# korentomas/mlx-mcmc

Measured on NVIDIA B200. Metric: leapfrog_grad_evals_per_sec, higher is better.
Workload: dtype f32

## Files before the change

mlx_mcmc_b200/csrc/glm_rows.cuh:

```cuda
#pragma once
#include "glm.cuh"

namespace b2m {

__host__ __device__ inline float pow2_scale(float m) {
  if (!(m > 0.f) || !(m < 3.0e38f)) return 1.0f;
  int e;
  frexpf(m, &e);
  int k = 14 - e;
  if (k > 100) k = 100;
  if (k < -100) k = -100;
  return ldexpf(1.0f, k);
}

__device__ __forceinline__ void split_f16(float v, __half &hi, __half &lo) {
  hi = __float2half_rn(v);
  lo = __float2half_rn(v - __half2float(hi));
}

struct PackP {
  const float *beta0;
  const int *tf;
  float *thc;
  int Dtot, beta_off, D, Dp, sigma_param;
  float sigma_const, weight;
  const float *inv_col_scale;
  const unsigned *y0max_bits;
  float x_rownorm_max;
  int logit;
  __half *Bh, *Bl;
  float *inv_var, *a_unscale, *r_scale, *r_unscale;
  int n_peers;
  __half *peer_Bh[kMaxPeers], *peer_Bl[kMaxPeers];
  float4 *peer_meta[kMaxPeers];
};

__device__ __forceinline__ void pack16_row(const PackP &P, const float *__restrict__ th, int64_t row, int lane) {
  const bool live = th != nullptr;
  B2M_ASSERT(row >= 0 && P.Dp % 64 == 0 && P.D <= P.Dp && P.beta_off + P.D <= P.Dtot);
  const int *tf = P.tf;
  float amax = 0.f, n2 = 0.f;
  if (live) {
    if (tf) {
      float *tc = P.thc + row * P.Dtot;
      for (int d = lane; d < P.Dtot; d += 32) tc[d] = tf_constrain(tf[d], th[d]);
      __syncwarp();
      th = tc;
    }
    for (int d = lane; d < P.D; d += 32) {
      const float dl = __fsub_rn(th[P.beta_off + d], P.beta0[d]);
      amax = fmaxf(amax, fabsf(dl * P.inv_col_scale[d]));
      n2 = fmaf(dl, dl, n2);
    }
  }
  for (int o = 16; o > 0; o >>= 1) {
    amax = fmaxf(amax, __shfl_xor_sync(0xffffffffu, amax, o));
    n2 += __shfl_xor_sync(0xffffffffu, n2, o);
  }
  const float sa = pow2_scale(amax);
  const float sg = (live && P.sigma_param >= 0) ? th[P.sigma_param] : P.sigma_const;
  const float iv = 1.0f / (sg * sg);
  if (P.n_peers == 0) {
    for (int d = lane; d < P.Dp; d += 32) {
      float v = 0.f;
      if (live && d < P.D) v = __fsub_rn(th[P.beta_off + d], P.beta0[d]) * P.inv_col_scale[d] * sa;
      __half hi, lo;
      split_f16(v, hi, lo);
      P.Bh[row * P.Dp + d] = hi;
      P.Bl[row * P.Dp + d] = lo;
    }
    if (lane == 0) {
      P.inv_var[row] = iv;
      P.a_unscale[row] = 1.0f / sa;
      if (P.r_scale) {
        const float bound = P.logit ? fabsf(P.weight)
                                    : (__uint_as_float(*P.y0max_bits) + sqrtf(n2) * P.x_rownorm_max) * fabsf(iv * P.weight);
        const float sr = pow2_scale(bound);
        P.r_scale[row] = sr;
        P.r_unscale[row] = 1.0f / sr;
      }
    }
  } else {
    for (int d = 2 * lane; d < P.Dp; d += 64) {
      float v0 = 0.f, v1 = 0.f;
      if (live && d < P.D) v0 = __fsub_rn(th[P.beta_off + d], P.beta0[d]) * P.inv_col_scale[d] * sa;
      if (live && d + 1 < P.D) v1 = __fsub_rn(th[P.beta_off + d + 1], P.beta0[d + 1]) * P.inv_col_scale[d + 1] * sa;
      const __half2 hi = __floats2half2_rn(v0, v1);
      const float2 hf = __half22float2(hi);
      const __half2 lo = __floats2half2_rn(v0 - hf.x, v1 - hf.y);
#pragma unroll
      for (int s = 0; s < kMaxPeers; ++s)
        if (s < P.n_peers) {
          *reinterpret_cast<__half2 *>(P.peer_Bh[s] + row * P.Dp + d) = hi;
          *reinterpret_cast<__half2 *>(P.peer_Bl[s] + row * P.Dp + d) = lo;
        }
    }
    if (lane < P.n_peers) P.peer_meta[lane][row] = make_float4(iv, 1.0f / sa, n2, 0.f);
  }
}

struct FinishP {
  int has_prior;
  int Dtot, beta_off, D, Dp, sigma_param;
  float sigma_const, weight;
  int N;
  int logit;
  int n_tiles;
  const float *ss_part;
  const float *G;
  int g_splits;
  int64_t Cp;
  const float *r_unscale;
  const float *inv_col_scale;
  const int *tf;
  const float *thc;
  int gram;
  const double *gb;
  const float *beta0;
  const float *a_unscale;
  const float *g_unscale;
};

__device__ __forceinline__ float gram_row(const FinishP &F, const float *__restrict__ th, int64_t c, float ivw,
                                          float *__restrict__ gr, int lane) {
  const int D = F.D, Dp = F.Dp, beta_off = F.beta_off;
  const int64_t stride = F.Cp * (int64_t)Dp;
  const float *__restrict__ Gr = F.G + c * Dp;
  const float au = F.a_unscale ? F.a_unscale[c] : 1.0f;
  const int step = (D & 3) == 0 ? 4 : 1;
  double acc = 0.0;
  for (int j0 = step * lane; j0 < D; j0 += 32 * step) {
    float p[4] = {0.f, 0.f, 0.f, 0.f};
    if (step == 4) {
#pragma unroll 4
      for (int s = 0; s < F.g_splits; ++s) {
        const float4 t = *reinterpret_cast<const float4 *>(Gr + s * stride + j0);
        p[0] += t.x; p[1] += t.y; p[2] += t.z; p[3] += t.w;
      }
    } else {
#pragma unroll 4
      for (int s = 0; s < F.g_splits; ++s) p[0] += Gr[s * stride + j0];
    }
#pragma unroll
    for (int e = 0; e < 4; ++e) {
      if (e >= step) break;
      const int j = j0 + e;
      const float pj = F.g_unscale ? p[e] * (au * F.g_unscale[j]) : p[e];
      const double bj = F.gb[j];
      const float dl = __fsub_rn(th[beta_off + j], F.beta0[j]);
      acc += (double)dl * ((double)pj - 2.0 * bj);
      if (gr) gr[beta_off + j] = (float)(bj - (double)pj) * ivw;
    }
  }
  for (int o = 16; o > 0; o >>= 1) acc += __shfl_xor_sync(0xffffffffu, acc, o);
  return (float)(F.gb[Dp] + acc);
}

__device__ __forceinline__ void finish_row(const FinishP &F, const SModel &sm, const float *__restrict__ th, int64_t c,
                                           int64_t c_batch, float *__restrict__ logp_out, float *__restrict__ gr, int lane) {
  B2M_ASSERT(c >= 0 && c < F.Cp && F.g_splits >= 0 && F.n_tiles >= 1);
  const float *thu = th;
  if (F.tf) th = F.thc + c_batch * F.Dtot;
  const int Dtot = F.Dtot, D = F.D, Dp = F.Dp, beta_off = F.beta_off, sigma_param = F.sigma_param;
  const int64_t Cp = F.Cp;
  const float *__restrict__ G = F.G;
  const float sg = sigma_param >= 0 ? th[sigma_param] : F.sigma_const;
  const float iv = 1.0f / (sg * sg);
  const float weight = F.weight;
  float ss = 0.f;
  if (F.gram) {
    ss = gram_row(F, th, c, iv * weight, gr, lane);
    if (gr) {
      for (int d = lane; d < Dtot; d += 32)
        if (d < beta_off || d >= beta_off + D) gr[d] = d == sigma_param ? weight * (ss * iv - (float)F.N) / sg : 0.f;
    }
    __syncwarp();
  } else {
    for (int t = lane; t < F.n_tiles; t += 32) ss += F.ss_part[(int64_t)t * Cp + c];
    for (int o = 16; o > 0; o >>= 1) ss += __shfl_xor_sync(0xffffffffu, ss, o);
  }
  float lp = F.logit ? weight * ss : weight * ((float)F.N * (-kHalfLog2Pi - logf(sg)) - 0.5f * ss * iv);
  const bool vec4 = !F.gram && gr && sigma_param < 0 && (Dtot & 3) == 0 && (beta_off & 3) == 0 && (D & 3) == 0 &&
                    ((reinterpret_cast<uintptr_t>(gr) | reinterpret_cast<uintptr_t>(G)) & 15) == 0;
  if (vec4) {
    const float ru = F.r_unscale ? F.r_unscale[c] : 1.0f;
    for (int d = 4 * lane; d < Dtot; d += 128) {
      float4 v = make_float4(0.f, 0.f, 0.f, 0.f);
      if (d >= beta_off && d < beta_off + D) {
        const float4 *g4 = reinterpret_cast<const float4 *>(G + (int64_t)c * Dp + (d - beta_off));
        const int64_t stride4 = (Cp * (int64_t)Dp) >> 2;
#pragma unroll 8
        for (int s = 0; s < F.g_splits; ++s) {
          const float4 t = g4[(int64_t)s * stride4];
          v.x += t.x; v.y += t.y; v.z += t.z; v.w += t.w;
        }
        if (F.r_unscale) {
          const float4 ic = *reinterpret_cast<const float4 *>(F.inv_col_scale + (d - beta_off));
          v.x *= ru * ic.x; v.y *= ru * ic.y; v.z *= ru * ic.z; v.w *= ru * ic.w;
        }
      }
      *reinterpret_cast<float4 *>(gr + d) = v;
    }
    __syncwarp();
  } else if (gr && !F.gram) {
#pragma unroll 2
    for (int d = lane; d < Dtot; d += 32) {
      float v = 0.f;
      if (d >= beta_off && d < beta_off + D) {
#pragma unroll 8
        for (int s = 0; s < F.g_splits; ++s) v += G[((int64_t)s * Cp + c) * Dp + (d - beta_off)];
        if (F.r_unscale) v *= F.r_unscale[c] * F.inv_col_scale[d - beta_off];
      }
      if (d == sigma_param) v = weight * (ss * iv - (float)F.N) / sg;
      gr[d] = v;
    }
    __syncwarp();
  }
  float pl = 0.f;
  const int n_terms = F.has_prior ? sm.n_terms : 0;
  for (int t = 0; t < n_terms; ++t) {
    const b2m_term &T = sm.terms[t];
    float acc = 0.f, ax = 0.f, a0 = 0.f, a1 = 0.f;
    if (T.dist == B2M_NORMAL && T.x.kind == B2M_OP_PARAMVEC && T.p0.kind == B2M_OP_CONST && T.p1.kind == B2M_OP_CONST) {
      const float p0 = T.p0.c, p1 = T.p1.c, var = p1 * p1, base = -kHalfLog2Pi - logf(p1), w = T.weight;
      const float *__restrict__ xv = th + T.x.a;
      float *__restrict__ gv = gr ? gr + T.x.a : nullptr;
      if ((T.length & 3) == 0 && ((reinterpret_cast<uintptr_t>(xv) | reinterpret_cast<uintptr_t>(gv)) & 15) == 0) {
        for (int n = 4 * lane; n < T.length; n += 128) {
          const float4 x4 = *reinterpret_cast<const float4 *>(xv + n);
          const float z0 = x4.x - p0, z1 = x4.y - p0, z2 = x4.z - p0, z3 = x4.w - p0;
          acc += base - (0.5f * (z0 * z0)) / var;
          acc += base - (0.5f * (z1 * z1)) / var;
          acc += base - (0.5f * (z2 * z2)) / var;
          acc += base - (0.5f * (z3 * z3)) / var;
          if (gv) {
            float4 g4 = *reinterpret_cast<float4 *>(gv + n);
            g4.x += w * (-(z0 / var)); g4.y += w * (-(z1 / var)); g4.z += w * (-(z2 / var)); g4.w += w * (-(z3 / var));
            *reinterpret_cast<float4 *>(gv + n) = g4;
          }
        }
      } else {
#pragma unroll 4
        for (int n = lane; n < T.length; n += 32) {
          const float z = xv[n] - p0;
          acc += base - (0.5f * (z * z)) / var;
          if (gv) gv[n] += w * (-(z / var));
        }
      }
      for (int o = 16; o > 0; o >>= 1) acc += __shfl_xor_sync(0xffffffffu, acc, o);
      pl += w * acc;
      __syncwarp();
      continue;
    }
    for (int n = lane; n < T.length; n += 32) {
      const float x = op_fetch(T.x, n, th, 1, sm), p0 = op_fetch(T.p0, n, th, 1, sm), p1 = op_fetch(T.p1, n, th, 1, sm);
      Elem e = dist_eval<true>(T.dist, x, p0, p1, T.k0, T.k1, T.k2);
      acc += e.lp;
      if (gr) {
        if (T.x.kind == B2M_OP_PARAM) ax += e.dx; else if (T.x.kind == B2M_OP_PARAMVEC) gr[T.x.a + n] += T.weight * e.dx;
        if (T.p0.kind == B2M_OP_PARAM) a0 += e.d0; else if (T.p0.kind == B2M_OP_PARAMVEC) gr[T.p0.a + n] += T.weight * e.d0;
        if (T.p1.kind == B2M_OP_PARAM) a1 += e.d1; else if (T.p1.kind == B2M_OP_PARAMVEC) gr[T.p1.a + n] += T.weight * e.d1;
      }
    }
    for (int o = 16; o > 0; o >>= 1) {
      acc += __shfl_xor_sync(0xffffffffu, acc, o);
      ax += __shfl_xor_sync(0xffffffffu, ax, o);
      a0 += __shfl_xor_sync(0xffffffffu, a0, o);
      a1 += __shfl_xor_sync(0xffffffffu, a1, o);
    }
// ... 29 lines not shown
```

mlx_mcmc_b200/csrc/glm_samplers.cu:

```cuda
#include <stdlib.h>

#include <chrono>
#include <string>
#include <vector>

#include "glm_rows.cuh"

namespace b2m {

constexpr int WPB = 4;

__device__ __forceinline__ float warp_sum(float v) {
  for (int o = 16; o > 0; o >>= 1) v += __shfl_xor_sync(0xffffffffu, v, o);
  return v;
}

__device__ __forceinline__ void normals4(uint64_t seed, uint64_t gchain, uint32_t giter, int group, float out[4]) {
  const uint4 w = Philox::draw(seed, gchain, giter, 1u + (uint32_t)group);
  box_muller(w.x, w.y, out[0], out[1]);
  box_muller(w.z, w.w, out[2], out[3]);
}

__device__ __noinline__ void fill_momentum(float *p, int D, const float *inj, uint64_t seed, uint64_t gchain, uint32_t giter,
                                           uint4 w0, int lane, const float *__restrict__ im = nullptr) {
// ... 253 lines not shown
  layout(real);
  const unsigned grid = (unsigned)((C + WPB - 1) / WPB);
  int rc = glm_logp_grad(gm, a.theta, C, a.logp, nullptr, st, true);
  for (int it = 0; it < a.n_iter && !rc; ++it) {
    if (it > 0 && (it & 15) == 0) rc = glm_recenter(gm, a.theta, C, st);
    mh_propose_kernel<<<grid, 32 * WPB, 0, st>>>(a, qn, D, it);
    rc = glm_logp_grad(gm, qn, C, lpn, nullptr, st);
    mh_accept_kernel<<<grid, 32 * WPB, 0, st>>>(a, qn, lpn, D, it, gm.tf);
    g_launches += 2;
  }
  cudaError_t e = cudaStreamSynchronize(st);
  if (rc) return rc;
  B2M_CHECK_CUDA(e);
  B2M_CHECK_CUDA(cudaGetLastError());
  return 0;
}

struct NutsBufs {
  float *g, *fq, *fp, *fg;
  float *slots;
  int n_slots;
  int *lo, *hi, *cand;
  int *leaf_slot;
  int *sub_c;
  int *st_f, *st_c;
  float *lp, *clp, *h0, *log_slice, *flp, *sclp, *feps, *heps;
  int *n, *s, *v, *leaf, *building, *sub_n, *sub_na, *sub_s, *alpha_cnt, *depth;
  double *alpha_sum, *sub_alpha;
  float *st_clp;
  int *st_n, *st_na;
  double *st_alpha;
  int *n_active;
  int *active;
  float *alpha_it;
  double *eps_it;
  int *state;
  int *iter;
  int *fin;
  int *live;
  int *n_done;
  double *pool;
  const int *tf;
};

__device__ __noinline__ void vcopy(float *__restrict__ dst, const float *__restrict__ src, int D, int lane) {
  if ((D & 3) == 0 && ((reinterpret_cast<uintptr_t>(dst) | reinterpret_cast<uintptr_t>(src)) & 15) == 0) {
// ... 97 lines not shown
    W.feps[c] = (float)((double)v * eps);
    W.heps[c] = (float)(0.5 * ((double)v * eps));
    W.leaf[c] = 0;
    W.building[c] = 1;
  }
}

__global__ void __launch_bounds__(32 * WPB) nuts_doubling_begin_kernel(b2m_nuts_args A, NutsBufs W, int D, int it, int j) {
  CHAIN_PROLOGUE(A.n_chains)
  nuts_doubling_begin_dev(A, W, D, c, lane, it, j);
}

__device__ __forceinline__ void nuts_leaf_pre_dev(const b2m_nuts_args &A, const NutsBufs &W, int D, int64_t c, int lane) {
  if (!W.building[c]) return;
  const size_t o = (size_t)c * D;
  const float he = W.heps[c], fe = W.feps[c];
  float *__restrict__ fq = W.fq + o, *__restrict__ fp = W.fp + o;
  const int s = W.leaf_slot[c];
  const float *__restrict__ sq = slot_row(W, D, c, s, 0), *__restrict__ sp = slot_row(W, D, c, s, 1),
                            *__restrict__ sg = slot_row(W, D, c, s, 2);
  if (const float *__restrict__ im = A.inv_mass) {
#pragma unroll 4
    for (int d = lane; d < D; d += 32) {
      const float pv = __fadd_rn(sp[d], __fmul_rn(he, sg[d]));
      fp[d] = pv;
      fq[d] = __fadd_rn(sq[d], __fmul_rn(fe, im[d] * pv));
    }
    return;
  }
  if ((D & 3) == 0 && ((reinterpret_cast<uintptr_t>(fq) | reinterpret_cast<uintptr_t>(fp) | reinterpret_cast<uintptr_t>(sq) |
                        reinterpret_cast<uintptr_t>(sp) | reinterpret_cast<uintptr_t>(sg)) & 15) == 0) {
    for (int d = 4 * lane; d < D; d += 128) {
      const float4 g4 = *reinterpret_cast<const float4 *>(sg + d);
      float4 p4 = *reinterpret_cast<const float4 *>(sp + d), q4 = *reinterpret_cast<const float4 *>(sq + d);
      p4.x = __fadd_rn(p4.x, __fmul_rn(he, g4.x)); p4.y = __fadd_rn(p4.y, __fmul_rn(he, g4.y));
      p4.z = __fadd_rn(p4.z, __fmul_rn(he, g4.z)); p4.w = __fadd_rn(p4.w, __fmul_rn(he, g4.w));
      q4.x = __fadd_rn(q4.x, __fmul_rn(fe, p4.x)); q4.y = __fadd_rn(q4.y, __fmul_rn(fe, p4.y));
      q4.z = __fadd_rn(q4.z, __fmul_rn(fe, p4.z)); q4.w = __fadd_rn(q4.w, __fmul_rn(fe, p4.w));
      *reinterpret_cast<float4 *>(fp + d) = p4;
      *reinterpret_cast<float4 *>(fq + d) = q4;
    }
    return;
  }
#pragma unroll 4
  for (int d = lane; d < D; d += 32) {
    const float pv = __fadd_rn(sp[d], __fmul_rn(he, sg[d]));
    fp[d] = pv;
    fq[d] = __fadd_rn(sq[d], __fmul_rn(fe, pv));
  }
}

__global__ void __launch_bounds__(32 * WPB) nuts_leaf_pre_kernel(b2m_nuts_args A, NutsBufs W, int D) {
  CHAIN_PROLOGUE(A.n_chains)
  nuts_leaf_pre_dev(A, W, D, c, lane);
}

__device__ __forceinline__ void nuts_leaf_post_dev(const b2m_nuts_args &A, const NutsBufs &W, int D, int64_t c, int lane, int it, int j) {
  if (!W.building[c]) return;
  const int64_t C = A.n_chains;
  const uint64_t gchain = (uint64_t)(A.chain_offset + c);
  const uint32_t giter = (uint32_t)(A.iter_offset + it);
  const size_t row = (size_t)it * C + c;
  const size_t o = (size_t)c * D;
  const int MD = A.max_tree_depth;
  const bool ref_compat = A.compat == B2M_COMPAT_REFERENCE;
  const float *fq = W.fq + o, *fp = W.fp + o, *fg = W.fg + o;
  const float he = W.heps[c];
  const int i = W.leaf[c];
  unsigned live = (1u << W.lo[c]) | (1u << W.hi[c]) | (1u << W.cand[c]);
  for (int k = 0; k < j; ++k)
    if ((i >> k) & 1) live |= (1u << W.st_f[(size_t)k * C + c]) | (1u << W.st_c[(size_t)k * C + c]);
  const int L = __ffs(~live) - 1;
  B2M_ASSERT(L >= 0 && L < W.n_slots);
  float *__restrict__ lq = slot_row(W, D, c, L, 0), *__restrict__ lp = slot_row(W, D, c, L, 1), *__restrict__ lg = slot_row(W, D, c, L, 2);
  float k0 = 0.f, k1 = 0.f;
  {
    int d = lane;
    if ((D & 3) == 0 && ((reinterpret_cast<uintptr_t>(fq) | reinterpret_cast<uintptr_t>(fp) | reinterpret_cast<uintptr_t>(fg) |
                          reinterpret_cast<uintptr_t>(lq) | reinterpret_cast<uintptr_t>(lp) | reinterpret_cast<uintptr_t>(lg)) & 15) == 0) {
      for (int e = 4 * lane; e < D; e += 128) {
        const float4 q4 = *reinterpret_cast<const float4 *>(fq + e), g4 = *reinterpret_cast<const float4 *>(fg + e);
        float4 p4 = *reinterpret_cast<const float4 *>(fp + e);
        p4.x = __fadd_rn(p4.x, __fmul_rn(he, g4.x)); p4.y = __fadd_rn(p4.y, __fmul_rn(he, g4.y));
        p4.z = __fadd_rn(p4.z, __fmul_rn(he, g4.z)); p4.w = __fadd_rn(p4.w, __fmul_rn(he, g4.w));
        k0 = fmaf(p4.x, p4.x, k0); k1 = fmaf(p4.y, p4.y, k1); k0 = fmaf(p4.z, p4.z, k0); k1 = fmaf(p4.w, p4.w, k1);
        *reinterpret_cast<float4 *>(lq + e) = q4; *reinterpret_cast<float4 *>(lp + e) = p4; *reinterpret_cast<float4 *>(lg + e) = g4;
      }
      d = D;
    }
    for (; d + 32 < D; d += 64) {
      const float q0 = fq[d], q1 = fq[d + 32], g0 = fg[d], g1 = fg[d + 32];
      const float p0 = __fadd_rn(fp[d], __fmul_rn(he, g0)), p1 = __fadd_rn(fp[d + 32], __fmul_rn(he, g1));
      k0 = fmaf(p0, p0, k0); k1 = fmaf(p1, p1, k1);
      lq[d] = q0; lq[d + 32] = q1; lp[d] = p0; lp[d + 32] = p1; lg[d] = g0; lg[d + 32] = g1;
    }
    for (; d < D; d += 32) {
      const float q0 = fq[d], g0 = fg[d];
      const float p0 = __fadd_rn(fp[d], __fmul_rn(he, g0));
      k0 = fmaf(p0, p0, k0);
      lq[d] = q0; lp[d] = p0; lg[d] = g0;
    }
  }
  float kin = 0.5f * warp_sum(k0 + k1);
  __syncwarp();
  if (A.inv_mass) kin = kinetic_w(lp, D, lane, A.inv_mass);
  const float flp = W.flp[c], h0 = W.h0[c], log_slice = W.log_slice[c];
  const float h1 = -flp + kin;
  const int n1 = (log_slice <= -h1) ? 1 : 0;
  const bool s1 = log_slice < (1000.0f - h1);
  float a1 = expf(-h1 + h0);
  if (a1 != a1) a1 = ref_compat ? 1.0f : 0.0f;
  a1 = fminf(a1, 1.0f);
  const int v = W.v[c];
  B2M_ASSERT(j >= 0 && j < A.max_tree_depth && i >= 0 && i < (1 << j) && (v == 1 || v == -1));
  if (lane == 0) {
    A.n_leaves[c] += 1;
    if (!s1) A.n_diverge[c] += 1;
  }
  float sub_clp = flp;
  int sub_n = n1, sub_na = 1;
  bool sub_s = s1;
  double sub_alpha = (double)a1;
  int sf = L, sc = L;
  int k = 0;
  bool finished = false;
  while (true) {
    if (k == j) { finished = true; break; }
    const size_t ss = (size_t)k * C + c;
// ... 27 lines not shown
    } else {
      if (sub_s) {
        if (lane == 0) {
          W.st_f[ss] = sf; W.st_c[ss] = sc;
          W.st_clp[ss] = sub_clp; W.st_n[ss] = sub_n; W.st_na[ss] = sub_na; W.st_alpha[ss] = sub_alpha;
        }
        break;
      }
      ++k;
    }
  }
  if (lane == 0) {
    W.leaf_slot[c] = L;
    if (finished) {
      W.building[c] = 0;
      W.sub_c[c] = sc;
      W.sclp[c] = sub_clp; W.sub_n[c] = sub_n; W.sub_na[c] = sub_na; W.sub_s[c] = sub_s ? 1 : 0; W.sub_alpha[c] = sub_alpha;
    } else {
      W.leaf[c] = i + 1;
    }
  }
}

__global__ void __launch_bounds__(32 * WPB) nuts_leaf_post_kernel(b2m_nuts_args A, NutsBufs W, int D, int it, int j) {
  CHAIN_PROLOGUE(A.n_chains)
  nuts_leaf_post_dev(A, W, D, c, lane, it, j);
}

__device__ __forceinline__ void nuts_doubling_end_dev(const b2m_nuts_args &A, const NutsBufs &W, int D, int64_t c, int lane, int it, int j) {
  if (!W.s[c]) return;
  const uint64_t gchain = (uint64_t)(A.chain_offset + c);
  const uint32_t giter = (uint32_t)(A.iter_offset + it);
  const size_t row = (size_t)it * A.n_chains + c;
  const int v = W.v[c];
  int lo = W.lo[c], hi = W.hi[c];
  if (v == 1) hi = W.leaf_slot[c];
  else        lo = W.leaf_slot[c];
  const int sub_n = W.sub_n[c], sub_s = W.sub_s[c];
  const int n = W.n[c];
  int took = 0;
  if (sub_s) {
    float ut;
    if (A.inj_take) ut = A.inj_take[row * A.max_tree_depth + j];
    else ut = u01(Philox::draw(A.seed, gchain, giter, SLOT_NUTS_DOUBLING + j).y);
    const double pr = fmin(1.0, (double)sub_n / fmax((double)n, 1.0));
    if ((double)ut < pr) took = 1;
// ... 110 lines not shown
    h_bar = (1.0 - eta) * h_bar + eta * (A.target_accept - mean_alpha);
    float log_eps = __fsub_rn(mu, (float)((sqrt(m + 1.0) / 0.05) * h_bar));
    log_eps = fmaxf(fminf(log_eps, 10.0f), -10.0f);
    const double eps = (double)expf(log_eps);
    const double wgt = pow(m + 1.0, -0.75);
    eps_bar = (double)expf((float)(wgt * log(eps) + (1.0 - wgt) * log(eps_bar)));
    eps_sh = eps; hbar_sh = h_bar; ebar_sh = eps_bar;
  }
  __syncthreads();
  for (int64_t c = threadIdx.x; c < C; c += 1024) {
    A.step_size[c] = eps_sh;
    A.da_state[c * 3 + 0] = hbar_sh;
    A.da_state[c * 3 + 1] = ebar_sh;
  }
}

static void nuts_layout(Arena &A, NutsBufs &W, int64_t C, int D, int MD) {
  const size_t cd = (size_t)C * D;
  float **vecs[] = {&W.g, &W.fq, &W.fp, &W.fg};
  for (auto v : vecs) A.take(v, cd);
  static_assert(2 * B2M_MAX_TREE_DEPTH + 2 <= 32, "the free-slot search keeps the live slots in a 32-bit mask");
  W.n_slots = 2 * MD + 2;
  A.take(&W.slots, cd * 3 * W.n_slots);
  float **fs[] = {&W.lp, &W.clp, &W.h0, &W.log_slice, &W.flp, &W.sclp, &W.feps, &W.heps};
  for (auto v : fs) A.take(v, C);
  int **is[] = {&W.n, &W.s, &W.v, &W.leaf, &W.building, &W.sub_n, &W.sub_na, &W.sub_s, &W.alpha_cnt, &W.depth,
                &W.lo, &W.hi, &W.cand, &W.leaf_slot, &W.sub_c};
  for (auto v : is) A.take(v, C);
  A.take(&W.st_f, (size_t)C * MD); A.take(&W.st_c, (size_t)C * MD);
  A.take(&W.alpha_sum, C); A.take(&W.sub_alpha, C);
  A.take(&W.st_clp, (size_t)C * MD); A.take(&W.st_n, (size_t)C * MD); A.take(&W.st_na, (size_t)C * MD);
  A.take(&W.st_alpha, (size_t)C * MD);
  A.take(&W.n_active, 1);
  A.take(&W.active, C);
  A.take(&W.alpha_it, C);
  A.take(&W.eps_it, C);
  A.take(&W.state, C); A.take(&W.iter, C); A.take(&W.fin, C); A.take(&W.live, C);
  A.take(&W.n_done, 1);
  A.take(&W.pool, 4);
}

__device__ __forceinline__ void nuts_tick_dev(const b2m_nuts_args &A, const NutsBufs &W, int D, int64_t c, int lane) {
  B2M_ASSERT(c >= 0 && c < A.n_chains);
  const int st = W.state[c];
  B2M_ASSERT(st >= 0 && st <= 2);
  if (st == 2) return;
  int it = W.iter[c];
  B2M_ASSERT(it >= 0 && it < A.n_iter);
  B2M_ASSERT(W.depth[c] >= 0 && W.depth[c] <= A.max_tree_depth);
  bool begin_transition = st == 0;
  int begin_doubling = -1;
  if (st != 0) {
    const int j = W.depth[c];
    nuts_leaf_post_dev(A, W, D, c, lane, it, j);
    __syncwarp();
    if (!W.building[c]) {
      nuts_doubling_end_dev(A, W, D, c, lane, it, j);
      __syncwarp();
      if (W.s[c] && W.depth[c] < A.max_tree_depth) {
        begin_doubling = W.depth[c];
      } else {
        nuts_end_dev(A, W, D, c, lane, it);
        __syncwarp();
        ++it;
        if (lane == 0) { W.iter[c] = it; W.fin[c] = 1; }
        if (it >= A.n_iter) {
          if (lane == 0) { W.state[c] = 2; W.live[c] = 0; atomicAdd(W.n_done, 1); }
          return;
        }
        begin_transition = true;
      }
    }
  }
  if (begin_transition) {
    nuts_begin_dev(A, W, D, c, lane, it);
    __syncwarp();
    begin_doubling = 0;
    if (st == 0 && lane == 0) W.state[c] = 1;
  }
  if (begin_doubling >= 0) {
    nuts_doubling_begin_dev(A, W, D, c, lane, it, begin_doubling);
    __syncwarp();
  }
  nuts_leaf_pre_dev(A, W, D, c, lane);
}

__global__ void __launch_bounds__(32 * WPB) nuts_tick_kernel(b2m_nuts_args A, NutsBufs W, int D, int64_t c_base, int64_t c_end) {
  const int lane = threadIdx.x & 31;
  const int64_t c = c_base + (int64_t)blockIdx.x * WPB + (threadIdx.x >> 5);
  if (c >= c_end) return;
  nuts_tick_dev(A, W, D, c, lane);
}

struct StateP {
  FinishP F;
  PackP P;
  const int *idx;
  int64_t n_rows;
  int64_t n_pad;
  int64_t row_base;
  int do_finish, do_tick_pack;
  unsigned *blk_counter;
  volatile long long *h_prog;
  long long tick;
  int peer, nranks, rank;
  unsigned long long wait_seq, seq;
  const unsigned long long *gflag;
  unsigned long long *bflag_peer[kMaxPeers];
  long long *done_peer[kMaxPeers];
  int *err;
};

constexpr int kProgRing = 8;
constexpr long long kSpinTimeout = 20000000000ll;

__device__ __forceinline__ unsigned long long ld_acquire_sys(const unsigned long long *p) {
  unsigned long long v;
  asm volatile("ld.acquire.sys.global.u64 %0, [%1];" : "=l"(v) : "l"(p) : "memory");
  return v;
}
__device__ __forceinline__ void st_release_sys(unsigned long long *p, unsigned long long v) {
  asm volatile("st.release.sys.global.u64 [%0], %1;" ::"l"(p), "l"(v) : "memory");
}
__device__ __forceinline__ void spin_until(const unsigned long long *flag, unsigned long long want, int *err) {
  const long long t0 = clock64();
  while (ld_acquire_sys(flag) < want) {
    if (*reinterpret_cast<volatile int *>(err)) return;
    if (clock64() - t0 > kSpinTimeout) { *reinterpret_cast<volatile int *>(err) = 1; __threadfence_system(); return; }
    __nanosleep(64);
  }
}

__global__ void __launch_bounds__(32 * WPB, 7) nuts_state_kernel(b2m_nuts_args A, NutsBufs W, int D, KModel prior, StateP S) {
  extern __shared__ __align__(16) unsigned char smem[];
  SModel sm;
  sm.n_terms = 0;
  if (S.do_finish && S.F.has_prior) model_to_smem(prior, smem, sm);
  const int lane = threadIdx.x & 31, warp = threadIdx.x >> 5;
  if (S.peer && S.do_finish) {
    if ((int)threadIdx.x < S.nranks) spin_until(S.gflag + threadIdx.x, S.wait_seq, S.err);
    __syncthreads();
  }
  const int64_t r = (int64_t)blockIdx.x * WPB + warp;
  if (r < S.n_rows) {
    const int64_t row = S.row_base + r;
    const int64_t c = S.idx ? S.idx[row] : row;
    B2M_ASSERT(c >= 0 && c < A.n_chains && row >= 0 && (S.peer || row < S.n_pad));
    if (S.do_finish) {
      finish_row(S.F, sm, W.fq + c * D, S.peer ? r : row, row, W.flp + c, W.fg + c * D, lane);
      __syncwarp();
    }
    if (S.do_tick_pack) {
      nuts_tick_dev(A, W, D, c, lane);
      __syncwarp();
      pack16_row(S.P, W.fq + c * D, row, lane);
    }
  } else if (r < S.n_pad && S.do_tick_pack) {
    pack16_row(S.P, nullptr, S.row_base + r, lane);
  }
  if (!S.do_tick_pack) return;
  if (S.peer) __threadfence_system(); else __threadfence();
  __syncwarp();
  int last_warp = 0;
  if (lane == 0) {
    const unsigned prev = atomicAdd(S.blk_counter, 1u);
    last_warp = prev == gridDim.x * WPB - 1;
    if (last_warp) *S.blk_counter = 0;
  }
  last_warp = __shfl_sync(0xffffffffu, last_warp, 0);
  if (!last_warp) return;
  __threadfence();
  const long long n_done = *reinterpret_cast<volatile int *>(W.n_done);
  if (S.peer) {
    if (lane < S.nranks) {
      *reinterpret_cast<volatile long long *>(S.done_peer[lane]) = n_done;
      __threadfence_system();
      st_release_sys(S.bflag_peer[lane], S.seq);
    }
// ... 495 lines not shown
```

Baseline: 31.65 million.

## Fuse NUTS leaf close into gradient finish and leaf open into pack

After: 36.45 million (median of 6 runs). 1.15x the previous value.

```diff
diff --git a/mlx_mcmc_b200/csrc/glm_rows.cuh b/mlx_mcmc_b200/csrc/glm_rows.cuh
--- a/mlx_mcmc_b200/csrc/glm_rows.cuh
+++ b/mlx_mcmc_b200/csrc/glm_rows.cuh
@@ -17,6 +17,16 @@
   hi = __float2half_rn(v);
   lo = __float2half_rn(v - __half2float(hi));
 }
+
+__device__ __forceinline__ float leaf_kick(float p, float he, float g) { return __fadd_rn(p, __fmul_rn(he, g)); }
+__device__ __forceinline__ float leaf_drift(float q, float fe, float v) { return __fadd_rn(q, __fmul_rn(fe, v)); }
+__device__ __forceinline__ float pack_coef(float th, float b0, float ics, float sa) { return __fsub_rn(th, b0) * ics * sa; }
+__device__ __forceinline__ float gram_elem(float pj, double bj, float dl, float ivw, double &acc) {
+  acc += (double)dl * ((double)pj - 2.0 * bj);
+  return (float)(bj - (double)pj) * ivw;
+}
+__device__ __forceinline__ float normal_prior_lp(float z, float base, float var) { return base - (0.5f * (z * z)) / var; }
+__device__ __forceinline__ float normal_prior_dx(float z, float var, float w) { return w * (-(z / var)); }
 
 struct PackP {
   const float *beta0;
@@ -63,7 +73,7 @@
   if (P.n_peers == 0) {
     for (int d = lane; d < P.Dp; d += 32) {
       float v = 0.f;
-      if (live && d < P.D) v = __fsub_rn(th[P.beta_off + d], P.beta0[d]) * P.inv_col_scale[d] * sa;
+      if (live && d < P.D) v = pack_coef(th[P.beta_off + d], P.beta0[d], P.inv_col_scale[d], sa);
       __half hi, lo;
       split_f16(v, hi, lo);
       P.Bh[row * P.Dp + d] = hi;
@@ -83,8 +93,8 @@
   } else {
     for (int d = 2 * lane; d < P.Dp; d += 64) {
       float v0 = 0.f, v1 = 0.f;
-      if (live && d < P.D) v0 = __fsub_rn(th[P.beta_off + d], P.beta0[d]) * P.inv_col_scale[d] * sa;
-      if (live && d + 1 < P.D) v1 = __fsub_rn(th[P.beta_off + d + 1], P.beta0[d + 1]) * P.inv_col_scale[d + 1] * sa;
+      if (live && d < P.D) v0 = pack_coef(th[P.beta_off + d], P.beta0[d], P.inv_col_scale[d], sa);
+      if (live && d + 1 < P.D) v1 = pack_coef(th[P.beta_off + d + 1], P.beta0[d + 1], P.inv_col_scale[d + 1], sa);
       const __half2 hi = __floats2half2_rn(v0, v1);
       const float2 hf = __half22float2(hi);
       const __half2 lo = __floats2half2_rn(v0 - hf.x, v1 - hf.y);
@@ -96,6 +106,55 @@
         }
     }
     if (lane < P.n_peers) P.peer_meta[lane][row] = make_float4(iv, 1.0f / sa, n2, 0.f);
+  }
+}
+
+__device__ __forceinline__ bool open_pack_ok(const PackP &P, int Dtot) {
+  return P.n_peers == 0 && !P.r_scale && !P.tf && P.sigma_param < 0 && P.beta_off == 0 && P.D == Dtot && (Dtot & 3) == 0 &&
+         ((reinterpret_cast<uintptr_t>(P.beta0) | reinterpret_cast<uintptr_t>(P.inv_col_scale)) & 15) == 0;
+}
+
+__device__ __forceinline__ void open_pack16_row(const PackP &P, const float *__restrict__ sq, const float *__restrict__ sp,
+                                                const float *__restrict__ sg, float he, float fe, float *__restrict__ q,
+                                                float *__restrict__ p, int64_t row, int lane) {
+  const int D = P.D;
+  float amax = 0.f;
+  for (int d = 4 * lane; d < D; d += 128) {
+    const float4 g4 = *reinterpret_cast<const float4 *>(sg + d), b4 = *reinterpret_cast<const float4 *>(P.beta0 + d),
+                 c4 = *reinterpret_cast<const float4 *>(P.inv_col_scale + d);
+    float4 p4 = *reinterpret_cast<const float4 *>(sp + d), q4 = *reinterpret_cast<const float4 *>(sq + d);
+    p4.x = leaf_kick(p4.x, he, g4.x); p4.y = leaf_kick(p4.y, he, g4.y);
+    p4.z = leaf_kick(p4.z, he, g4.z); p4.w = leaf_kick(p4.w, he, g4.w);
+    q4.x = leaf_drift(q4.x, fe, p4.x); q4.y = leaf_drift(q4.y, fe, p4.y);
+    q4.z = leaf_drift(q4.z, fe, p4.z); q4.w = leaf_drift(q4.w, fe, p4.w);
+    *reinterpret_cast<float4 *>(p + d) = p4;
+    *reinterpret_cast<float4 *>(q + d) = q4;
+    amax = fmaxf(amax, fabsf(__fsub_rn(q4.x, b4.x) * c4.x)); amax = fmaxf(amax, fabsf(__fsub_rn(q4.y, b4.y) * c4.y));
+    amax = fmaxf(amax, fabsf(__fsub_rn(q4.z, b4.z) * c4.z)); amax = fmaxf(amax, fabsf(__fsub_rn(q4.w, b4.w) * c4.w));
+  }
+  for (int o = 16; o > 0; o >>= 1) amax = fmaxf(amax, __shfl_xor_sync(0xffffffffu, amax, o));
+  const float sa = pow2_scale(amax);
+  for (int d = 4 * lane; d < P.Dp; d += 128) {
+    float v[4] = {0.f, 0.f, 0.f, 0.f};
+    if (d < D) {
+      const float4 q4 = *reinterpret_cast<const float4 *>(q + d), b4 = *reinterpret_cast<const float4 *>(P.beta0 + d),
+                   c4 = *reinterpret_cast<const float4 *>(P.inv_col_scale + d);
+      v[0] = pack_coef(q4.x, b4.x, c4.x, sa); v[1] = pack_coef(q4.y, b4.y, c4.y, sa);
+      v[2] = pack_coef(q4.z, b4.z, c4.z, sa); v[3] = pack_coef(q4.w, b4.w, c4.w, sa);
+    }
+    __half hi[4], lo[4];
+#pragma unroll
+    for (int e = 0; e < 4; ++e) split_f16(v[e], hi[e], lo[e]);
+    *reinterpret_cast<uint2 *>(P.Bh + row * P.Dp + d) =
+        make_uint2(__half_as_ushort(hi[0]) | (unsigned)__half_as_ushort(hi[1]) << 16,
+                   __half_as_ushort(hi[2]) | (unsigned)__half_as_ushort(hi[3]) << 16);
+    *reinterpret_cast<uint2 *>(P.Bl + row * P.Dp + d) =
+        make_uint2(__half_as_ushort(lo[0]) | (unsigned)__half_as_ushort(lo[1]) << 16,
+                   __half_as_ushort(lo[2]) | (unsigned)__half_as_ushort(lo[3]) << 16);
+  }
+  if (lane == 0) {
+    P.inv_var[row] = 1.0f / (P.sigma_const * P.sigma_const);
+    P.a_unscale[row] = 1.0f / sa;
   }
 }
 
@@ -121,6 +180,10 @@
   const float *g_unscale;
 };
 
+__device__ __forceinline__ float gram_unscale(const FinishP &F, float pj, float au, int j) {
+  return F.g_unscale ? pj * (au * F.g_unscale[j]) : pj;
+}
+
 __device__ __forceinline__ float gram_row(const FinishP &F, const float *__restrict__ th, int64_t c, float ivw,
                                           float *__restrict__ gr, int lane) {
   const int D = F.D, Dp = F.Dp, beta_off = F.beta_off;
@@ -145,15 +208,74 @@
     for (int e = 0; e < 4; ++e) {
       if (e >= step) break;
       const int j = j0 + e;
-      const float pj = F.g_unscale ? p[e] * (au * F.g_unscale[j]) : p[e];
-      const double bj = F.gb[j];
-      const float dl = __fsub_rn(th[beta_off + j], F.beta0[j]);
-      acc += (double)dl * ((double)pj - 2.0 * bj);
-      if (gr) gr[beta_off + j] = (float)(bj - (double)pj) * ivw;
+      const float g = gram_elem(gram_unscale(F, p[e], au, j), F.gb[j], __fsub_rn(th[beta_off + j], F.beta0[j]), ivw, acc);
+      if (gr) gr[beta_off + j] = g;
     }
   }
   for (int o = 16; o > 0; o >>= 1) acc += __shfl_xor_sync(0xffffffffu, acc, o);
   return (float)(F.gb[Dp] + acc);
+}
+
+__device__ __forceinline__ float lik_value(const FinishP &F, float ss, float sg, float iv) {
+  return F.logit ? F.weight * ss : F.weight * ((float)F.N * (-kHalfLog2Pi - logf(sg)) - 0.5f * ss * iv);
+}
+
+__device__ __forceinline__ bool normal_const_term(const b2m_term &T) {
+  return T.dist == B2M_NORMAL && T.x.kind == B2M_OP_PARAMVEC && T.p0.kind == B2M_OP_CONST && T.p1.kind == B2M_OP_CONST;
+}
+
+__device__ __forceinline__ bool close_fast_ok(const FinishP &F, const SModel &sm) {
+  if (!F.gram || F.logit || F.tf || F.sigma_param >= 0 || F.beta_off != 0 || F.D != F.Dtot || (F.D & 3) != 0 ||
+      !F.has_prior || sm.n_terms != 1 || !normal_const_term(sm.terms[0]))
+    return false;
+  return sm.terms[0].x.a == 0 && sm.terms[0].length == F.D;
+}
+
+__device__ __forceinline__ float close_row_gram_normal(const FinishP &F, const b2m_term &T, const float *__restrict__ q,
+                                                       const float *__restrict__ p, float he, int64_t c, float *__restrict__ lq,
+                                                       float *__restrict__ lp, float *__restrict__ lg, float &k0, float &k1,
+                                                       int lane) {
+  const int D = F.D, Dp = F.Dp;
+  const int64_t stride = F.Cp * (int64_t)Dp;
+  const float *__restrict__ Gr = F.G + c * Dp;
+  const float au = F.a_unscale ? F.a_unscale[c] : 1.0f;
+  const float sg = F.sigma_const;
+  const float iv = 1.0f / (sg * sg);
+  const float ivw = iv * F.weight;
+  const float p0 = T.p0.c, p1 = T.p1.c, var = p1 * p1, base = -kHalfLog2Pi - logf(p1), w = T.weight;
+  double acc = 0.0;
+  float pacc = 0.f;
+  for (int j0 = 4 * lane; j0 < D; j0 += 128) {
+    float s[4] = {0.f, 0.f, 0.f, 0.f};
+#pragma unroll 4
+    for (int k = 0; k < F.g_splits; ++k) {
+      const float4 t = *reinterpret_cast<const float4 *>(Gr + k * stride + j0);
+      s[0] += t.x; s[1] += t.y; s[2] += t.z; s[3] += t.w;
+    }
+    const float4 q4 = *reinterpret_cast<const float4 *>(q + j0), p4 = *reinterpret_cast<const float4 *>(p + j0);
+    const float x[4] = {q4.x, q4.y, q4.z, q4.w}, pv[4] = {p4.x, p4.y, p4.z, p4.w};
+    float g[4], pn[4];
+#pragma unroll
+    for (int e = 0; e < 4; ++e) {
+      const int j = j0 + e;
+      g[e] = gram_elem(gram_unscale(F, s[e], au, j), F.gb[j], __fsub_rn(x[e], F.beta0[j]), ivw, acc);
+      const float z = x[e] - p0;
+      pacc += normal_prior_lp(z, base, var);
+      g[e] += normal_prior_dx(z, var, w);
+      pn[e] = leaf_kick(pv[e], he, g[e]);
+    }
+    k0 = fmaf(pn[0], pn[0], k0); k1 = fmaf(pn[1], pn[1], k1); k0 = fmaf(pn[2], pn[2], k0); k1 = fmaf(pn[3], pn[3], k1);
+    *reinterpret_cast<float4 *>(lq + j0) = q4;
+    *reinterpret_cast<float4 *>(lp + j0) = make_float4(pn[0], pn[1], pn[2], pn[3]);
+    *reinterpret_cast<float4 *>(lg + j0) = make_float4(g[0], g[1], g[2], g[3]);
+  }
+  for (int o = 16; o > 0; o >>= 1) acc += __shfl_xor_sync(0xffffffffu, acc, o);
+  for (int o = 16; o > 0; o >>= 1) pacc += __shfl_xor_sync(0xffffffffu, pacc, o);
+  const float ss = (float)(F.gb[Dp] + acc);
+  const float lp_lik = lik_value(F, ss, sg, iv);
+  float pl = 0.f, lj = 0.f;
+  pl += w * pacc;
+  return lp_lik + pl + lj;
 }
 
 __device__ __forceinline__ void finish_row(const FinishP &F, const SModel &sm, const float *__restrict__ th, int64_t c,
@@ -179,7 +301,7 @@
     for (int t = lane; t < F.n_tiles; t += 32) ss += F.ss_part[(int64_t)t * Cp + c];
     for (int o = 16; o > 0; o >>= 1) ss += __shfl_xor_sync(0xffffffffu, ss, o);
   }
-  float lp = F.logit ? weight * ss : weight * ((float)F.N * (-kHalfLog2Pi - logf(sg)) - 0.5f * ss * iv);
+  float lp = lik_value(F, ss, sg, iv);
   const bool vec4 = !F.gram && gr && sigma_param < 0 && (Dtot & 3) == 0 && (beta_off & 3) == 0 && (D & 3) == 0 &&
                     ((reinterpret_cast<uintptr_t>(gr) | reinterpret_cast<uintptr_t>(G)) & 15) == 0;
   if (vec4) {
@@ -221,30 +343,33 @@
   for (int t = 0; t < n_terms; ++t) {
     const b2m_term &T = sm.terms[t];
     float acc = 0.f, ax = 0.f, a0 = 0.f, a1 = 0.f;
-    if (T.dist == B2M_NORMAL && T.x.kind == B2M_OP_PARAMVEC && T.p0.kind == B2M_OP_CONST && T.p1.kind == B2M_OP_CONST) {
+    if (normal_const_term(T)) {
       const float p0 = T.p0.c, p1 = T.p1.c, var = p1 * p1, base = -kHalfLog2Pi - logf(p1), w = T.weight;
       const float *__restrict__ xv = th + T.x.a;
       float *__restrict__ gv = gr ? gr + T.x.a : nullptr;
-      if ((T.length & 3) == 0 && ((reinterpret_cast<uintptr_t>(xv) | reinterpret_cast<uintptr_t>(gv)) & 15) == 0) {
+      if ((T.length & 3) == 0 && (reinterpret_cast<uintptr_t>(xv) & 15) == 0) {
+        const bool gv4 = (reinterpret_cast<uintptr_t>(gv) & 15) == 0;
         for (int n = 4 * lane; n < T.length; n += 128) {
           const float4 x4 = *reinterpret_cast<const float4 *>(xv + n);
-          const float z0 = x4.x - p0, z1 = x4.y - p0, z2 = x4.z - p0, z3 = x4.w - p0;
-          acc += base - (0.5f * (z0 * z0)) / var;
-          acc += base - (0.5f * (z1 * z1)) / var;
-          acc += base - (0.5f * (z2 * z2)) / var;
-          acc += base - (0.5f * (z3 * z3)) / var;
-          if (gv) {
+          const float z[4] = {x4.x - p0, x4.y - p0, x4.z - p0, x4.w - p0};
+#pragma unroll
+          for (int e = 0; e < 4; ++e) acc += normal_prior_lp(z[e], base, var);
+          if (gv && gv4) {
             float4 g4 = *reinterpret_cast<float4 *>(gv + n);
-            g4.x += w * (-(z0 / var)); g4.y += w * (-(z1 / var)); g4.z += w * (-(z2 / var)); g4.w += w * (-(z3 / var));
+            g4.x += normal_prior_dx(z[0], var, w); g4.y += normal_prior_dx(z[1], var, w);
+            g4.z += normal_prior_dx(z[2], var, w); g4.w += normal_prior_dx(z[3], var, w);
             *reinterpret_cast<float4 *>(gv + n) = g4;
+          } else if (gv) {
+#pragma unroll
+            for (int e = 0; e < 4; ++e) gv[n + e] += normal_prior_dx(z[e], var, w);
           }
         }
       } else {
 #pragma unroll 4
         for (int n = lane; n < T.length; n += 32) {
           const float z = xv[n] - p0;
-          acc += base - (0.5f * (z * z)) / var;
-          if (gv) gv[n] += w * (-(z / var));
+          acc += normal_prior_lp(z, base, var);
+          if (gv) gv[n] += normal_prior_dx(z, var, w);
         }
       }
       for (int o = 16; o > 0; o >>= 1) acc += __shfl_xor_sync(0xffffffffu, acc, o);
diff --git a/mlx_mcmc_b200/csrc/glm_samplers.cu b/mlx_mcmc_b200/csrc/glm_samplers.cu
--- a/mlx_mcmc_b200/csrc/glm_samplers.cu
+++ b/mlx_mcmc_b200/csrc/glm_samplers.cu
@@ -299,6 +299,8 @@
   int n_slots;
   int *lo, *hi, *cand;
   int *leaf_slot;
+  int *leaf_new;
+  float *leaf_kin;
   int *sub_c;
   int *st_f, *st_c;
   float *lp, *clp, *h0, *log_slice, *flp, *sclp, *feps, *heps;
@@ -442,9 +444,9 @@
   if (const float *__restrict__ im = A.inv_mass) {
 #pragma unroll 4
     for (int d = lane; d < D; d += 32) {
-      const float pv = __fadd_rn(sp[d], __fmul_rn(he, sg[d]));
+      const float pv = leaf_kick(sp[d], he, sg[d]);
       fp[d] = pv;
-      fq[d] = __fadd_rn(sq[d], __fmul_rn(fe, im[d] * pv));
+      fq[d] = leaf_drift(sq[d], fe, im[d] * pv);
     }
     return;
   }
@@ -453,10 +455,10 @@
     for (int d = 4 * lane; d < D; d += 128) {
       const float4 g4 = *reinterpret_cast<const float4 *>(sg + d);
       float4 p4 = *reinterpret_cast<const float4 *>(sp + d), q4 = *reinterpret_cast<const float4 *>(sq + d);
-      p4.x = __fadd_rn(p4.x, __fmul_rn(he, g4.x)); p4.y = __fadd_rn(p4.y, __fmul_rn(he, g4.y));
-      p4.z = __fadd_rn(p4.z, __fmul_rn(he, g4.z)); p4.w = __fadd_rn(p4.w, __fmul_rn(he, g4.w));
-      q4.x = __fadd_rn(q4.x, __fmul_rn(fe, p4.x)); q4.y = __fadd_rn(q4.y, __fmul_rn(fe, p4.y));
-      q4.z = __fadd_rn(q4.z, __fmul_rn(fe, p4.z)); q4.w = __fadd_rn(q4.w, __fmul_rn(fe, p4.w));
+      p4.x = leaf_kick(p4.x, he, g4.x); p4.y = leaf_kick(p4.y, he, g4.y);
+      p4.z = leaf_kick(p4.z, he, g4.z); p4.w = leaf_kick(p4.w, he, g4.w);
+      q4.x = leaf_drift(q4.x, fe, p4.x); q4.y = leaf_drift(q4.y, fe, p4.y);
+      q4.z = leaf_drift(q4.z, fe, p4.z); q4.w = leaf_drift(q4.w, fe, p4.w);
       *reinterpret_cast<float4 *>(fp + d) = p4;
       *reinterpret_cast<float4 *>(fq + d) = q4;
     }
@@ -464,9 +466,9 @@
   }
 #pragma unroll 4
   for (int d = lane; d < D; d += 32) {
-    const float pv = __fadd_rn(sp[d], __fmul_rn(he, sg[d]));
+    const float pv = leaf_kick(sp[d], he, sg[d]);
     fp[d] = pv;
-    fq[d] = __fadd_rn(sq[d], __fmul_rn(fe, pv));
+    fq[d] = leaf_drift(sq[d], fe, pv);
   }
 }
 
@@ -475,55 +477,68 @@
   nuts_leaf_pre_dev(A, W, D, c, lane);
 }
 
-__device__ __forceinline__ void nuts_leaf_post_dev(const b2m_nuts_args &A, const NutsBufs &W, int D, int64_t c, int lane, int it, int j) {
-  if (!W.building[c]) return;
-  const int64_t C = A.n_chains;
-  const uint64_t gchain = (uint64_t)(A.chain_offset + c);
-  const uint32_t giter = (uint32_t)(A.iter_offset + it);
-  const size_t row = (size_t)it * C + c;
-  const size_t o = (size_t)c * D;
-  const int MD = A.max_tree_depth;
-  const bool ref_compat = A.compat == B2M_COMPAT_REFERENCE;
-  const float *fq = W.fq + o, *fp = W.fp + o, *fg = W.fg + o;
-  const float he = W.heps[c];
+__device__ __forceinline__ int nuts_leaf_slot(const NutsBufs &W, int64_t C, int64_t c, int j) {
   const int i = W.leaf[c];
   unsigned live = (1u << W.lo[c]) | (1u << W.hi[c]) | (1u << W.cand[c]);
   for (int k = 0; k < j; ++k)
     if ((i >> k) & 1) live |= (1u << W.st_f[(size_t)k * C + c]) | (1u << W.st_c[(size_t)k * C + c]);
   const int L = __ffs(~live) - 1;
   B2M_ASSERT(L >= 0 && L < W.n_slots);
-  float *__restrict__ lq = slot_row(W, D, c, L, 0), *__restrict__ lp = slot_row(W, D, c, L, 1), *__restrict__ lg = slot_row(W, D, c, L, 2);
+  return L;
+}
+
+__device__ __forceinline__ float nuts_leaf_store_dev(const b2m_nuts_args &A, const NutsBufs &W, int D, int64_t c, int L,
+                                                     const float *g, int lane) {
+  const size_t o = (size_t)c * D;
+  const float *fq = W.fq + o, *fp = W.fp + o;
+  const float he = W.heps[c];
+  float *__restrict__ lq = slot_row(W, D, c, L, 0), *__restrict__ lp = slot_row(W, D, c, L, 1), *lg = slot_row(W, D, c, L, 2);
+  const bool store_g = g != lg;
   float k0 = 0.f, k1 = 0.f;
-  {
-    int d = lane;
-    if ((D & 3) == 0 && ((reinterpret_cast<uintptr_t>(fq) | reinterpret_cast<uintptr_t>(fp) | reinterpret_cast<uintptr_t>(fg) |
-                          reinterpret_cast<uintptr_t>(lq) | reinterpret_cast<uintptr_t>(lp) | reinterpret_cast<uintptr_t>(lg)) & 15) == 0) {
-      for (int e = 4 * lane; e < D; e += 128) {
-        const float4 q4 = *reinterpret_cast<const float4 *>(fq + e), g4 = *reinterpret_cast<const float4 *>(fg + e);
-        float4 p4 = *reinterpret_cast<const float4 *>(fp + e);
-        p4.x = __fadd_rn(p4.x, __fmul_rn(he, g4.x)); p4.y = __fadd_rn(p4.y, __fmul_rn(he, g4.y));
-        p4.z = __fadd_rn(p4.z, __fmul_rn(he, g4.z)); p4.w = __fadd_rn(p4.w, __fmul_rn(he, g4.w));
-        k0 = fmaf(p4.x, p4.x, k0); k1 = fmaf(p4.y, p4.y, k1); k0 = fmaf(p4.z, p4.z, k0); k1 = fmaf(p4.w, p4.w, k1);
-        *reinterpret_cast<float4 *>(lq + e) = q4; *reinterpret_cast<float4 *>(lp + e) = p4; *reinterpret_cast<float4 *>(lg + e) = g4;
-      }
-      d = D;
-    }
-    for (; d + 32 < D; d += 64) {
-      const float q0 = fq[d], q1 = fq[d + 32], g0 = fg[d], g1 = fg[d + 32];
-      const float p0 = __fadd_rn(fp[d], __fmul_rn(he, g0)), p1 = __fadd_rn(fp[d + 32], __fmul_rn(he, g1));
-      k0 = fmaf(p0, p0, k0); k1 = fmaf(p1, p1, k1);
-      lq[d] = q0; lq[d + 32] = q1; lp[d] = p0; lp[d + 32] = p1; lg[d] = g0; lg[d + 32] = g1;
-    }
-    for (; d < D; d += 32) {
-      const float q0 = fq[d], g0 = fg[d];
-      const float p0 = __fadd_rn(fp[d], __fmul_rn(he, g0));
-      k0 = fmaf(p0, p0, k0);
-      lq[d] = q0; lp[d] = p0; lg[d] = g0;
-    }
+  int d = lane;
+  if ((D & 3) == 0 && ((reinterpret_cast<uintptr_t>(fq) | reinterpret_cast<uintptr_t>(fp) | reinterpret_cast<uintptr_t>(g) |
+                        reinterpret_cast<uintptr_t>(lq) | reinterpret_cast<uintptr_t>(lp) | reinterpret_cast<uintptr_t>(lg)) & 15) == 0) {
+    for (int e = 4 * lane; e < D; e += 128) {
+      const float4 q4 = *reinterpret_cast<const float4 *>(fq + e), g4 = *reinterpret_cast<const float4 *>(g + e);
+      float4 p4 = *reinterpret_cast<const float4 *>(fp + e);
+      p4.x = leaf_kick(p4.x, he, g4.x); p4.y = leaf_kick(p4.y, he, g4.y);
+      p4.z = leaf_kick(p4.z, he, g4.z); p4.w = leaf_kick(p4.w, he, g4.w);
+      k0 = fmaf(p4.x, p4.x, k0); k1 = fmaf(p4.y, p4.y, k1); k0 = fmaf(p4.z, p4.z, k0); k1 = fmaf(p4.w, p4.w, k1);
+      *reinterpret_cast<float4 *>(lq + e) = q4; *reinterpret_cast<float4 *>(lp + e) = p4;
+      if (store_g) *reinterpret_cast<float4 *>(lg + e) = g4;
+    }
+    d = D;
+  }
+  for (; d + 32 < D; d += 64) {
+    const float q0 = fq[d], q1 = fq[d + 32], g0 = g[d], g1 = g[d + 32];
+    const float p0 = leaf_kick(fp[d], he, g0), p1 = leaf_kick(fp[d + 32], he, g1);
+    k0 = fmaf(p0, p0, k0); k1 = fmaf(p1, p1, k1);
+    lq[d] = q0; lq[d + 32] = q1; lp[d] = p0; lp[d + 32] = p1;
+    if (store_g) { lg[d] = g0; lg[d + 32] = g1; }
+  }
+  for (; d < D; d += 32) {
+    const float q0 = fq[d], g0 = g[d];
+    const float p0 = leaf_kick(fp[d], he, g0);
+    k0 = fmaf(p0, p0, k0);
+    lq[d] = q0; lp[d] = p0;
+    if (store_g) lg[d] = g0;
   }
   float kin = 0.5f * warp_sum(k0 + k1);
   __syncwarp();
   if (A.inv_mass) kin = kinetic_w(lp, D, lane, A.inv_mass);
+  return kin;
+}
+
+__device__ __forceinline__ void nuts_leaf_tree_dev(const b2m_nuts_args &A, const NutsBufs &W, int D, int64_t c, int lane, int it,
+                                                   int j, int L, float kin) {
+  const int64_t C = A.n_chains;
+  const uint64_t gchain = (uint64_t)(A.chain_offset + c);
+  const uint32_t giter = (uint32_t)(A.iter_offset + it);
+  const size_t row = (size_t)it * C + c;
+  const int MD = A.max_tree_depth;
+  const bool ref_compat = A.compat == B2M_COMPAT_REFERENCE;
+  const int i = W.leaf[c];
+  const float *lq = slot_row(W, D, c, L, 0), *lp = slot_row(W, D, c, L, 1);
   const float flp = W.flp[c], h0 = W.h0[c], log_slice = W.log_slice[c];
   const float h1 = -flp + kin;
   const int n1 = (log_slice <= -h1) ? 1 : 0;
@@ -597,6 +612,13 @@
   }
 }
 
+__device__ __forceinline__ void nuts_leaf_post_dev(const b2m_nuts_args &A, const NutsBufs &W, int D, int64_t c, int lane, int it, int j) {
+  if (!W.building[c]) return;
+  const int L = nuts_leaf_slot(W, A.n_chains, c, j);
+  const float kin = nuts_leaf_store_dev(A, W, D, c, L, W.fg + (size_t)c * D, lane);
+  nuts_leaf_tree_dev(A, W, D, c, lane, it, j, L, kin);
+}
+
 __global__ void __launch_bounds__(32 * WPB) nuts_leaf_post_kernel(b2m_nuts_args A, NutsBufs W, int D, int it, int j) {
   CHAIN_PROLOGUE(A.n_chains)
   nuts_leaf_post_dev(A, W, D, c, lane, it, j);
@@ -753,10 +775,10 @@
   static_assert(2 * B2M_MAX_TREE_DEPTH + 2 <= 32, "the free-slot search keeps the live slots in a 32-bit mask");
   W.n_slots = 2 * MD + 2;
   A.take(&W.slots, cd * 3 * W.n_slots);
-  float **fs[] = {&W.lp, &W.clp, &W.h0, &W.log_slice, &W.flp, &W.sclp, &W.feps, &W.heps};
+  float **fs[] = {&W.lp, &W.clp, &W.h0, &W.log_slice, &W.flp, &W.sclp, &W.feps, &W.heps, &W.leaf_kin};
   for (auto v : fs) A.take(v, C);
   int **is[] = {&W.n, &W.s, &W.v, &W.leaf, &W.building, &W.sub_n, &W.sub_na, &W.sub_s, &W.alpha_cnt, &W.depth,
-                &W.lo, &W.hi, &W.cand, &W.leaf_slot, &W.sub_c};
+                &W.lo, &W.hi, &W.cand, &W.leaf_slot, &W.sub_c, &W.leaf_new};
   for (auto v : is) A.take(v, C);
   A.take(&W.st_f, (size_t)C * MD); A.take(&W.st_c, (size_t)C * MD);
   A.take(&W.alpha_sum, C); A.take(&W.sub_alpha, C);
@@ -771,11 +793,12 @@
   A.take(&W.pool, 4);
 }
 
-__device__ __forceinline__ void nuts_tick_dev(const b2m_nuts_args &A, const NutsBufs &W, int D, int64_t c, int lane) {
+template <bool kClosed>
+__device__ __forceinline__ bool nuts_tick_dev(const b2m_nuts_args &A, const NutsBufs &W, int D, int64_t c, int lane) {
   B2M_ASSERT(c >= 0 && c < A.n_chains);
   const int st = W.state[c];
   B2M_ASSERT(st >= 0 && st <= 2);
-  if (st == 2) return;
+  if (st == 2) return false;
   int it = W.iter[c];
   B2M_ASSERT(it >= 0 && it < A.n_iter);
   B2M_ASSERT(W.depth[c] >= 0 && W.depth[c] <= A.max_tree_depth);
@@ -783,7 +806,12 @@
   int begin_doubling = -1;
   if (st != 0) {
     const int j = W.depth[c];
-    nuts_leaf_post_dev(A, W, D, c, lane, it, j);
+    if (!kClosed) {
+      nuts_leaf_post_dev(A, W, D, c, lane, it, j);
+    } else {
+      B2M_ASSERT(W.building[c]);
+      nuts_leaf_tree_dev(A, W, D, c, lane, it, j, W.leaf_new[c], W.leaf_kin[c]);
+    }
     __syncwarp();
     if (!W.building[c]) {
       nuts_doubling_end_dev(A, W, D, c, lane, it, j);
@@ -797,7 +825,7 @@
         if (lane == 0) { W.iter[c] = it; W.fin[c] = 1; }
         if (it >= A.n_iter) {
           if (lane == 0) { W.state[c] = 2; W.live[c] = 0; atomicAdd(W.n_done, 1); }
-          return;
+          return false;
         }
         begin_transition = true;
       }
@@ -813,14 +841,14 @@
     nuts_doubling_begin_dev(A, W, D, c, lane, it, begin_doubling);
     __syncwarp();
   }
-  nuts_leaf_pre_dev(A, W, D, c, lane);
+  return true;
 }
 
 __global__ void __launch_bounds__(32 * WPB) nuts_tick_kernel(b2m_nuts_args A, NutsBufs W, int D, int64_t c_base, int64_t c_end) {
   const int lane = threadIdx.x & 31;
   const int64_t c = c_base + (int64_t)blockIdx.x * WPB + (threadIdx.x >> 5);
   if (c >= c_end) return;
-  nuts_tick_dev(A, W, D, c, lane);
+  if (nuts_tick_dev<false>(A, W, D, c, lane)) nuts_leaf_pre_dev(A, W, D, c, lane);
 }
 
 struct StateP {
@@ -842,6 +870,45 @@
   int *err;
 };
 
+__device__ __forceinline__ void nuts_leaf_close_dev(const b2m_nuts_args &A, const NutsBufs &W, int D, const FinishP &F,
+                                                    const SModel &sm, bool fast, int64_t c, int64_t c_f, int64_t row, int lane) {
+  if (!W.building[c]) return;
+  const int L = nuts_leaf_slot(W, A.n_chains, c, W.depth[c]);
+  const size_t o = (size_t)c * D;
+  const float *fq = W.fq + o, *fp = W.fp + o;
+  float *lq = slot_row(W, D, c, L, 0), *lp = slot_row(W, D, c, L, 1), *lg = slot_row(W, D, c, L, 2);
+  float kin;
+  if (fast && ((reinterpret_cast<uintptr_t>(fq) | reinterpret_cast<uintptr_t>(fp) | reinterpret_cast<uintptr_t>(lq) |
+                reinterpret_cast<uintptr_t>(lp) | reinterpret_cast<uintptr_t>(lg) | reinterpret_cast<uintptr_t>(F.G + c_f * F.Dp)) & 15) == 0) {
+    B2M_ASSERT(c_f >= 0 && c_f < F.Cp);
+    float k0 = 0.f, k1 = 0.f;
+    const float logp = close_row_gram_normal(F, sm.terms[0], fq, fp, W.heps[c], c_f, lq, lp, lg, k0, k1, lane);
+    if (lane == 0) W.flp[c] = logp;
+    kin = 0.5f * warp_sum(k0 + k1);
+    __syncwarp();
+    if (A.inv_mass) kin = kinetic_w(lp, D, lane, A.inv_mass);
+  } else {
+    finish_row(F, sm, fq, c_f, row, W.flp + c, lg, lane);
+    __syncwarp();
+    kin = nuts_leaf_store_dev(A, W, D, c, L, lg, lane);
+  }
+  if (lane == 0) { W.leaf_new[c] = L; W.leaf_kin[c] = kin; }
+}
+
+__device__ __forceinline__ bool nuts_leaf_open_pack_dev(const b2m_nuts_args &A, const NutsBufs &W, int D, const PackP &P,
+                                                        int64_t c, int64_t row, int lane) {
+  if (A.inv_mass || !open_pack_ok(P, D)) return false;
+  const size_t o = (size_t)c * D;
+  float *fq = W.fq + o, *fp = W.fp + o;
+  const int s = W.leaf_slot[c];
+  const float *sq = slot_row(W, D, c, s, 0), *sp = slot_row(W, D, c, s, 1), *sg = slot_row(W, D, c, s, 2);
+  if (((reinterpret_cast<uintptr_t>(fq) | reinterpret_cast<uintptr_t>(fp) | reinterpret_cast<uintptr_t>(sq) |
+        reinterpret_cast<uintptr_t>(sp) | reinterpret_cast<uintptr_t>(sg)) & 15) != 0)
+    return false;
+  open_pack16_row(P, sq, sp, sg, W.heps[c], W.feps[c], fq, fp, row, lane);
+  return true;
+}
+
 constexpr int kProgRing = 8;
 constexpr long long kSpinTimeout = 20000000000ll;
 
@@ -878,13 +945,19 @@
     const int64_t c = S.idx ? S.idx[row] : row;
     B2M_ASSERT(c >= 0 && c < A.n_chains && row >= 0 && (S.peer || row < S.n_pad));
     if (S.do_finish) {
-      finish_row(S.F, sm, W.fq + c * D, S.peer ? r : row, row, W.flp + c, W.fg + c * D, lane);
+      nuts_leaf_close_dev(A, W, D, S.F, sm, !S.peer && close_fast_ok(S.F, sm), c, S.peer ? r : row, row, lane);
       __syncwarp();
     }
     if (S.do_tick_pack) {
-      nuts_tick_dev(A, W, D, c, lane);
+      const bool open = nuts_tick_dev<true>(A, W, D, c, lane);
       __syncwarp();
-      pack16_row(S.P, W.fq + c * D, row, lane);
+      if (!(open && nuts_leaf_open_pack_dev(A, W, D, S.P, c, row, lane))) {
+        if (open) {
+          nuts_leaf_pre_dev(A, W, D, c, lane);
+          __syncwarp();
+        }
+        pack16_row(S.P, W.fq + c * D, row, lane);
+      }
     }
   } else if (r < S.n_pad && S.do_tick_pack) {
     pack16_row(S.P, nullptr, S.row_base + r, lane);
```
